# martinber/noaa-apt

Hardware: AMD Instinct MI355X
Metric: Msamples/sec WAV->APT-line decode (higher is better)
Workload: dtype f32; 1 GPU; synthetic 48000 Hz APT recording, 600 s (28800000 samples) per GPU, profile=standard: resample 13/50 (959 taps) -> AM envelope -> 37-tap low-pass -> sync correlation + peak picker -> 1198 rows x 2080 px; parallelism=1 GPU(s), 16 independent recordings per GPU and step, no collectives, recordings_per_call=16, mode=strict, rows=1198, n_sync=1199, input_resident_in_hbm=True, distinct_inputs_round_robin=16

## Files before the change

### noaa_apt_amd/csrc/apt_kernels_fused.hip

```cpp
#include "apt_kernels_fused_launch.hpp"

#include <hip/hip_runtime.h>

#include <cmath>
#include <cstdio>
#include <cstdlib>
#include <algorithm>
#include <cstring>
#include <type_traits>
#include <vector>

#pragma clang fp contract(off)

namespace apt::gpu {


bool fused_supported(uint32_t l, uint32_t m, uint32_t t1, uint32_t t2, uint32_t pw)
{
    if (l == 13 && m == 50 && t1 == 959 && t2 == 37 && pw == 3) return true;
    if (l == 13 && m == 100 && t1 == 1915 && t2 == 37 && pw == 3) return true;
    if (l == 13 && m == 30 && t1 == 2783 && t2 == 61 && pw == 5) return true;
    if (l == 13 && m == 60 && t1 == 5565 && t2 == 61 && pw == 5) return true;
    if (l == 13 && m == 75 && t1 == 639 && t2 == 43 && pw == 4) return true;
    return false;
}

uint32_t fused_group_size(uint32_t l) { return 4 * l; }

bool fused_takes_pcm16(uint32_t l, uint32_t m) { (void)l; return m % 2 == 0; }

uint32_t fused_tap_table_floats(uint32_t l, uint32_t m, uint32_t t1, int ch)
{
    (void)ch;
    const int li = static_cast<int>(l), mi = static_cast<int>(m), ti = static_cast<int>(t1);
    return static_cast<uint32_t>(fused_split_table_offset(li, mi, ti, 1) + (fused_split_nch(li, mi, ti, 1) + 1) * kSplitChunkDwords);
}

void fused_branch_taps(uint32_t l, uint32_t m, const float *coeff, uint32_t t1, int ch, float *hs, uint32_t t1_layout)
{
    (void)ch;
    if (t1_layout == 0) t1_layout = t1;
    const uint32_t tp = (t1_layout + l - 1) / l;
    const uint32_t clast = ((l - 1) * m + l - 1) / l;
    const uint32_t win = clast + tp;
    auto tap = [&](uint32_t b, int64_t q) -> float {
        const uint32_t cb = (b * m + l - 1) / l;
        const uint32_t pb = cb * l - b * m;
        if (q < static_cast<int64_t>(cb) || q >= static_cast<int64_t>(win)) return 0.f;
        const uint64_t j = pb + static_cast<uint64_t>(q - cb) * l;
        return j < t1 ? coeff[j] : 0.f;
    };
    const int li = static_cast<int>(l), mi = static_cast<int>(m), ti = static_cast<int>(t1_layout);
    for (int h = 0; h < 2; ++h) {
        const int b0 = fused_split_b0(li, h), nbr = fused_split_nbr(li, h), w0 = fused_split_w0(li, mi, h);
        const int nch_h = fused_split_nch(li, mi, ti, h);
        float *base = hs + fused_split_table_offset(li, mi, ti, h);
        for (int c = 0; c <= nch_h; ++c) {
            float *row = base + static_cast<size_t>(c) * kSplitChunkDwords;
            for (int i = 0; i < kSplitChunkDwords; ++i) row[i] = 0.f;
            if (c == nch_h) break;
            for (int e = 0; e < kSplitChunk; ++e) {
                const int64_t q = w0 + static_cast<int64_t>(kSplitChunk) * c + e;
                for (int k = 0; k < nbr / 2; ++k) {
                    row[6 * e + 2 * k] = tap(static_cast<uint32_t>(b0 + 2 * k), q);
                    row[6 * e + 2 * k + 1] = tap(static_cast<uint32_t>(b0 + 2 * k + 1), q);
                }
                if (nbr & 1) row[24 + e] = tap(static_cast<uint32_t>(b0 + nbr - 1), q);
            }
        }
    }
}

int fused_chunk_of(uint32_t m, bool fast)
{
    return fused_chunk(static_cast<int>(m), fast ? kModeFast : kModeStrict);
}

void fused_lowpass_pairs(const float *h2, uint32_t t2, float *h2p)
{
    for (uint32_t k = 0; k <= t2; ++k) {
        h2p[2 * k] = k >= 1 ? h2[k - 1] : 0.f;
        h2p[2 * k + 1] = k < t2 ? h2[k] : 0.f;
    }
}

uint32_t fused_f16_table_dwords(uint32_t l, uint32_t m, uint32_t t1)
{
    const uint32_t tp = (t1 + l - 1) / l;
    const uint32_t clast = ((l - 1) * m + l - 1) / l;
    return ((clast + tp + 1) / 2) * 16;
}

float fused_f16_branch_taps(uint32_t l, uint32_t m, const float *coeff, uint32_t t1, uint32_t *table)
{
    const uint32_t tp = (t1 + l - 1) / l;
    const uint32_t clast = ((l - 1) * m + l - 1) / l;
    const uint32_t win = clast + tp;
    auto tap = [&](uint32_t b, uint32_t q) -> float {
        const uint32_t cb = (b * m + l - 1) / l;
        const uint32_t pb = cb * l - b * m;
        if (q < cb || q >= win) return 0.f;
        const uint64_t j = pb + static_cast<uint64_t>(q - cb) * l;
        return j < t1 ? coeff[j] : 0.f;
    };
    float mx = 0.f;
    for (uint32_t j = 0; j < t1; ++j) mx = fmaxf(mx, fabsf(coeff[j]));
    int e = 0;
    if (mx > 0.f) (void)frexpf(mx, &e);
    const int sh = -e + 1;
    const float scale = ldexpf(1.f, sh);
    auto bits = [](float v) -> uint32_t {
        const _Float16 h = static_cast<_Float16>(v);
        uint16_t u;
        __builtin_memcpy(&u, &h, 2);
        return u;
    };
    const uint32_t nqp = (win + 1) / 2;
    for (uint32_t qp = 0; qp < nqp; ++qp)
        for (uint32_t b = 0; b < 16; ++b)
            table[qp * 16 + b] = b < l ? (bits(tap(b, 2 * qp) * scale) | (bits(tap(b, 2 * qp + 1) * scale) << 16)) : 0u;
    return ldexpf(1.f, -sh);
}

bool fused_f16_supported(uint32_t l, uint32_t m, uint32_t t1, uint32_t t2, uint32_t pw)
{
    return l == 13 && m == 50 && t1 == 959 && t2 == 37 && pw == 3;
}

float fused_gm_slack(uint32_t pw, float scale)
{
    return static_cast<float>(38u * pw - 1u + pw + 18u) * 1.03f * 0x1p-24f * 1.0001f * (scale >= 1.f ? scale : 1.f);
}

bool fused_fast_supported(uint32_t l, uint32_t m, uint32_t t1, uint32_t t2, uint32_t pw)
{
    if (l == 13 && m == 60 && t1 == 5565) return false;
    if (l == 13 && m == 75) return false;
    return fused_supported(l, m, t1, t2, pw);
}

uint32_t fused_pad_t2(uint32_t l, uint32_t m, uint32_t t2, uint32_t pw)
{
    if (l != 13 || pw != 3 || (m != 50 && m != 100)) return 0;
    if ((t2 & 1u) == 0 || t2 == 37 || t2 > static_cast<uint32_t>(kPadT2Max)) return 0;
    return static_cast<uint32_t>(kPadT2Max);
}
uint32_t fused_pad_t1(uint32_t l, uint32_t m, uint32_t t1, uint32_t t2, uint32_t pw)
{
    if (l != 13 || (t1 & 1u) == 0) return 0;
    uint32_t bound = 0;
    if ((t2 == 37 || fused_pad_t2(l, m, t2, pw) != 0) && pw == 3) bound = m == 50 ? kPadT1Max48k : m == 100 ? kPadT1Max96k : 0;
    else if (t2 == 61 && pw == 5) bound = m == 30 ? kPadT1Max48kSlow : m == 60 ? kPadT1Max96kSlow : 0;
    else if (t2 == 43 && pw == 4) bound = m == 75 ? kPadT1Max96kFastp : 0;
    return t1 <= bound ? bound : 0;
}

bool fused_mfma_supported(uint32_t l, uint32_t m, uint32_t t1, uint32_t t2, uint32_t pw)
{
    if (l != 13 || t2 != 37 || pw != 3 || (t1 & 1u) == 0) return false;
    if (m == 50) return t1 <= static_cast<uint32_t>(kMfmaT1Max48k);
    if (m == 100) return t1 <= static_cast<uint32_t>(kMfmaT1Max96k);
    return false;
}

namespace {
uint32_t mfma_kpad(uint32_t l, uint32_t m)
{
    const uint32_t t1max = m == 50 ? kMfmaT1Max48k : kMfmaT1Max96k;
    const uint32_t win = ((l - 1) * m + l - 1) / l + (t1max + l - 1) / l;
    return (win + 31u) / 32u * 32u;
}
template <typename At>
void mfma_fragments(At &&at, uint32_t nks, uint32_t *table)
{
    auto upper = [](float v) -> uint32_t {
        uint32_t u;
        __builtin_memcpy(&u, &v, 4);
        return u >> 16;
    };
    auto value = [](uint32_t h) -> float {
        const uint32_t u = h << 16;
        float v;
        __builtin_memcpy(&v, &u, 4);
        return v;
    };
    for (uint32_t s = 0; s < nks; ++s)
        for (uint32_t lane = 0; lane < 64; ++lane)
            for (uint32_t jp = 0; jp < 4; ++jp) {
                uint32_t w[3] = {0, 0, 0};
                for (uint32_t h = 0; h < 2; ++h) {
                    const float v = at(lane & 15u, 32u * s + 8u * (lane >> 4) + 2u * jp + h);
                    const uint32_t p0 = upper(v);
                    const float r1 = v - value(p0);
                    const uint32_t p1 = upper(r1);
                    const float r2 = r1 - value(p1);
                    const uint32_t p2 = upper(r2);
                    w[0] |= p0 << (16u * h);
                    w[1] |= p1 << (16u * h);
                    w[2] |= p2 << (16u * h);
                }
                for (uint32_t pc = 0; pc < 3; ++pc) table[((pc * nks + s) * 64u + lane) * 4u + jp] = w[pc];
            }
}
}

uint32_t fused_mfma_table_dwords(uint32_t l, uint32_t m) { return 3u * (mfma_kpad(l, m) / 32u) * 64u * 4u; }

void fused_mfma_table(uint32_t l, uint32_t m, const float *coeff, uint32_t t1, uint32_t *table)
{
    auto at = [&](uint32_t b, uint32_t q) -> float {
        if (b >= l) return 0.f;
        const uint32_t cb = (b * m + l - 1) / l, pb = cb * l - b * m;
        if (q < cb) return 0.f;
        const uint64_t j = pb + static_cast<uint64_t>(q - cb) * l;
        return j < t1 ? coeff[j] : 0.f;
    };
    mfma_fragments(at, mfma_kpad(l, m) / 32u, table);
}

bool fused_front_end(hipStream_t s, uint32_t l, uint32_t m, uint32_t t1, uint32_t t2, uint32_t pw, int mode,
                     bool pcm16, const CallArgs &call, const FusedParams *d_prm, uint64_t max_w, int lds_pad)
{
    if (call.count == 0 || call.count > static_cast<uint32_t>(kMaxCall)) return false;
// ... 479 lines not shown
```

### noaa_apt_amd/csrc/apt_kernels_fused_impl.hpp

```cpp
#pragma once

#include "apt_kernels_fused_launch.hpp"
#include "apt_envelope.hpp"
#include "apt_sync_corr.hpp"

#include <hip/hip_runtime.h>

#include <algorithm>
#include <atomic>
#include <cmath>
#include <cstdlib>
#include <type_traits>

#pragma clang fp contract(off)

#define APT_S1(n) "s" #n
#define APT_S8_(a, b, c, d, e, f, g, h) APT_S1(a), APT_S1(b), APT_S1(c), APT_S1(d), APT_S1(e), APT_S1(f), APT_S1(g), APT_S1(h)
#define APT_S8(n) APT_S8_X(n)
#define APT_S16(n) APT_S16_X(n)
#define APT_S8_X(n) APT_S8_##n
#define APT_S16_X(n) APT_S16_##n
#define APT_S8_52 APT_S8_(52, 53, 54, 55, 56, 57, 58, 59)
#define APT_S16_36 APT_S8_(36, 37, 38, 39, 40, 41, 42, 43), APT_S8_(44, 45, 46, 47, 48, 49, 50, 51)
#define APT_S16_64 APT_S8_(64, 65, 66, 67, 68, 69, 70, 71), APT_S8_(72, 73, 74, 75, 76, 77, 78, 79)
// ... 787 lines not shown
        for (int b = 0; b < L; ++b) r[b] = (kq + b < k_lo || kq + b >= k_hi) ? 0.f : acc[b] * f16_unscale;
    } else if constexpr (MFMA) {
        static_assert(Gm::SPLIT && L <= 16 && M % 2 == 0 && Gm::XSHIFT % 2 == 0, "windows start on sample pairs");
        constexpr int NS = Gm::NS, NKS = Gm::KPAD / 32, PLANE = Gm::XT_PAD / 2;
        constexpr int NGW = NS / 16 / (NTHR / 64);
        static_assert(NGW * 16 * (NTHR / 64) == NS, "whole groups per wave");
        uint32_t *l32 = reinterpret_cast<uint32_t *>(lds);
        uint32_t *nf_flag = l32 + 2 * PLANE;
        const int lane = tid & 63, wave = tid >> 6;
        typedef uint32_t u4m __attribute__((ext_vector_type(4)));
        typedef __bf16 b8m __attribute__((ext_vector_type(8)));
        auto as_b8 = [](u4m v) -> b8m { return __builtin_bit_cast(b8m, v); };
        typedef const u4m __attribute__((address_space(1))) *gu4_ptr;
        const gu4_ptr atab = (gu4_ptr)(prm->hs) + lane;
        if (tid == 0) *nf_flag = 0u;
        auto planes_to_lds = [&](const XReg (&xv)[NXR]) {
#pragma unroll
            for (int e = 0; e < NXR; ++e) {
                const int q = (tid + e * kFusedThreads) * 4;
                if (q < Gm::XT_PAD) {
                    float v[4];
                    if constexpr (sizeof(XT) == 4) {
                        v[0] = xv[e].x, v[1] = xv[e].y, v[2] = xv[e].z, v[3] = xv[e].w;
                    } else {
                        v[0] = static_cast<float>(static_cast<int16_t>(xv[e].x & 0xFFFFu)), v[1] = static_cast<float>(static_cast<int32_t>(xv[e].x) >> 16);
                        v[2] = static_cast<float>(static_cast<int16_t>(xv[e].y & 0xFFFFu)), v[3] = static_cast<float>(static_cast<int32_t>(xv[e].y) >> 16);
                    }
                    float r[4];
#pragma unroll
                    for (int i = 0; i < 4; ++i) r[i] = v[i] - __uint_as_float(__float_as_uint(v[i]) & 0xFFFF0000u);
                    const u2 w0 = (u2){__builtin_amdgcn_perm(__float_as_uint(v[1]), __float_as_uint(v[0]), 0x07060302u),
                                       __builtin_amdgcn_perm(__float_as_uint(v[3]), __float_as_uint(v[2]), 0x07060302u)};
                    const u2 w1 = (u2){__builtin_amdgcn_perm(__float_as_uint(r[1]), __float_as_uint(r[0]), 0x07060302u),
                                       __builtin_amdgcn_perm(__float_as_uint(r[3]), __float_as_uint(r[2]), 0x07060302u)};
                    *reinterpret_cast<u2 *>(l32 + q / 2) = w0;
                    *reinterpret_cast<u2 *>(l32 + PLANE + q / 2) = w1;
                }
            }
        };
        f4 racc[2][NGW];
        auto mfma_sub = [&](auto subc) {
            constexpr int SUB = decltype(subc)::value;
            int base[NGW];
#pragma unroll
            for (int g = 0; g < NGW; ++g) {
                racc[SUB][g] = (f4){0.f, 0.f, 0.f, 0.f};
                const int wl = (wave * NGW + g) * 16 + (lane & 15);
                base[g] = wl * (M / 2) + Gm::XSHIFT / 2 + 4 * (lane >> 4);
            }
            u4m an0 = atab[0], an1 = atab[NKS * 64], an2 = atab[2 * NKS * 64];
#pragma unroll
            for (int s_ = 0; s_ < NKS; ++s_) {
                const u4m a0 = an0, a1 = an1, a2 = an2;
                if (s_ + 1 < NKS) {
                    an0 = atab[(s_ + 1) * 64];
                    an1 = atab[(NKS + s_ + 1) * 64];
                    an2 = atab[(2 * NKS + s_ + 1) * 64];
                }
                u4m b0[NGW], b1[NGW];
#pragma unroll
                for (int g = 0; g < NGW; ++g) {
                    const uint32_t *bp = l32 + base[g] + 16 * s_;
                    b0[g] = (u4m){bp[0], bp[1], bp[2], bp[3]};
                    b1[g] = (u4m){bp[PLANE], bp[PLANE + 1], bp[PLANE + 2], bp[PLANE + 3]};
                }
#pragma unroll
                for (int g = 0; g < NGW; ++g) racc[SUB][g] = __builtin_amdgcn_mfma_f32_16x16x32_bf16(as_b8(a2), as_b8(b0[g]), racc[SUB][g], 0, 0, 0);
#pragma unroll
                for (int g = 0; g < NGW; ++g) racc[SUB][g] = __builtin_amdgcn_mfma_f32_16x16x32_bf16(as_b8(a1), as_b8(b1[g]), racc[SUB][g], 0, 0, 0);
#pragma unroll
                for (int g = 0; g < NGW; ++g) racc[SUB][g] = __builtin_amdgcn_mfma_f32_16x16x32_bf16(as_b8(a1), as_b8(b0[g]), racc[SUB][g], 0, 0, 0);
#pragma unroll
                for (int g = 0; g < NGW; ++g) racc[SUB][g] = __builtin_amdgcn_mfma_f32_16x16x32_bf16(as_b8(a0), as_b8(b1[g]), racc[SUB][g], 0, 0, 0);
#pragma unroll
                for (int g = 0; g < NGW; ++g) racc[SUB][g] = __builtin_amdgcn_mfma_f32_16x16x32_bf16(as_b8(a0), as_b8(b0[g]), racc[SUB][g], 0, 0, 0);
                __builtin_amdgcn_sched_barrier(0);
            }
        };
        XReg xr1[NXR];
        planes_to_lds(xr);
        __builtin_amdgcn_sched_barrier(0);
        load_tile(ri, tile, 1, xr1);
        __syncthreads();
        mfma_sub(std::integral_constant<int, 0>{});
        __syncthreads();
        planes_to_lds(xr1);
        __syncthreads();
        mfma_sub(std::integral_constant<int, 1>{});
        APT_MARK("END stage1");
        {
            float sum = 0.f;
#pragma unroll
            for (int sub = 0; sub < 2; ++sub)
#pragma unroll
                for (int g = 0; g < NGW; ++g) sum += (racc[sub][g].x + racc[sub][g].y) + (racc[sub][g].z + racc[sub][g].w);
            if ((__float_as_uint(sum) & 0x7F800000u) == 0x7F800000u) *nf_flag = 1u;
        }
        __syncthreads();
        const bool tile_nf = *nf_flag != 0u;
        {
#pragma unroll
            for (int sub = 0; sub < 2; ++sub)
#pragma unroll
                for (int g = 0; g < NGW; ++g) {
                    const int wdw = sub * NS + (wave * NGW + g) * 16 + (lane & 15);
#pragma unroll
                    for (int rr_ = 0; rr_ < 4; ++rr_) {
                        const int b = 4 * (lane >> 4) + rr_;
                        if (b < L) P[wdw * L + b] = racc[sub][g][rr_];
                    }
                }
        }
        if (tile_nf) {
            __syncthreads();
            const XT *__restrict__ xg = static_cast<const XT *>(call.rec[ri].x);
            const uint64_t n_in = call.rec[ri].n;
            const float *__restrict__ cf = prm->coeff;
            const uint32_t t1r = prm->t1;
            for (int b = 0; b < L; ++b) {
                const int64_t k = (tile * Gm::OWN_K - Gm::PRE_K) + kq + b;
                float sum = 0.f;
                if (k >= 0) {
                    const uint64_t v = static_cast<uint64_t>(k) * static_cast<uint64_t>(M);
                    uint64_t x0 = (v + L - 1) / L;
                    for (uint64_t j = x0 * L - v; j < t1r; j += L, ++x0)
                        if (x0 < n_in) sum = __builtin_fmaf(cf[j], static_cast<float>(xg[x0]), sum);
                }
                P[tid * L + b] = sum;
            }
        }
        __syncthreads();
#pragma unroll
        for (int b = 0; b < L; ++b) r[b] = P[tid * L + b];
        if (!interior) {
            bool any = false;
#pragma unroll
            for (int b = 0; b < L; ++b)
                if (kq + b < k_lo || kq + b >= k_hi) {
                    r[b] = 0.f;
                    any = true;
                }
            if (any) {
#pragma unroll
                for (int b = 0; b < L; ++b) P[tid * L + b] = r[b];
            }
            __syncthreads();
        }
    } else if constexpr (Gm::SPLIT) {
        static_assert(L == 13 && Gm::XSHIFT % 2 == 0 && (M % 2 == 0 || sizeof(XT) == 4),
                      "SPLIT: halves of 7 and 6 branches (three pairs each); window reads of aligned sample pairs, or — odd M, f32 input only — of single samples");
        constexpr bool WIDE = M % 4 == 0 && Gm::XSHIFT % 4 == 0;
        constexpr int NS = Gm::NS;
        const int wl = tid & (NS - 1);
        constexpr int NH0 = fused_split_nbr(L, 0);
        float rh[2][NH0];
        if constexpr (PAD) {
#pragma unroll
            for (int j = 0; j < NH0; ++j) rh[0][j] = rh[1][j] = 0.f;
        }
        auto half = [&](auto hc, auto subc) {
            constexpr int H = decltype(hc)::value, SUB = decltype(subc)::value;
            constexpr int B0 = fused_split_b0(L, H), NBR = fused_split_nbr(L, H);
            constexpr int NPH = NBR / 2;
            constexpr bool ODDH = (NBR & 1) != 0;
            static_assert(NPH == 3, "three branch pairs per half");
            constexpr int W0 = fused_split_w0(L, M, H), NCH = fused_split_nch(L, M, T1, H);
            constexpr int CHW = kSplitChunkDwords;
            const cf2_ptr hsp = hs + fused_split_table_offset(L, M, T1, H) / 2;
            typedef uint32_t u16s __attribute__((ext_vector_type(16)));
            typedef uint32_t u8s __attribute__((ext_vector_type(8)));
            typedef uint32_t u4s __attribute__((ext_vector_type(4)));
            u16s ta[2];
            u8s tb[2];
            u4s tc[2];
            typedef float f4w __attribute__((ext_vector_type(4)));
            using XRaw = std::conditional_t<sizeof(XT) == 4, f4w, u2>;
            XRaw xraw[2];
            f2 acc[NPH];
            float accl = 0.f;
#pragma unroll
            for (int k = 0; k < NPH; ++k) acc[k] = (f2){0.f, 0.f};
            auto issue = [&](auto cc) {
                constexpr int c = decltype(cc)::value;
                if constexpr ((c & 1) == 0)
                    asm volatile("s_load_dwordx16 s[36:51], %0, %1\n\ts_load_dwordx8 s[52:59], %0, %2\n\ts_load_dwordx4 s[60:63], %0, %3"
                                 :: "s"(hsp), "n"(c * CHW * 4), "n"(c * CHW * 4 + 64), "n"(c * CHW * 4 + 96)
                                 : APT_S16(36), APT_S8(52), APT_S4_60);
                else
                    asm volatile("s_load_dwordx16 s[64:79], %0, %1\n\ts_load_dwordx8 s[80:87], %0, %2\n\ts_load_dwordx4 s[88:91], %0, %3"
                                 :: "s"(hsp), "n"(c * CHW * 4), "n"(c * CHW * 4 + 64), "n"(c * CHW * 4 + 96)
                                 : APT_S16(64), APT_S8(80), APT_S4_88);
                constexpr int q0 = Gm::XSHIFT + W0 + kSplitChunk * c;
                if constexpr (sizeof(XT) == 4) {
                    if constexpr (WIDE) {
                        xraw[c & 1] = *reinterpret_cast<const f4w *>(P + wl * M + q0);
                    } else if constexpr (M % 2 != 0) {
                        const float *wp = P + wl * M + q0;
                        xraw[c & 1] = (f4w){wp[0], wp[1], wp[2], wp[3]};
                    } else {
                        const f2 lo = *reinterpret_cast<const f2 *>(P + wl * M + q0), hi = *reinterpret_cast<const f2 *>(P + wl * M + q0 + 2);
                        xraw[c & 1] = (f4w){lo.x, lo.y, hi.x, hi.y};
                    }
                } else if constexpr (WIDE) {
                    xraw[c & 1] = *reinterpret_cast<const u2 *>(reinterpret_cast<const int16_t *>(lds) + wl * M + q0);
                } else {
                    const uint32_t *w32 = reinterpret_cast<const uint32_t *>(lds) + (wl * M + q0) / 2;
                    xraw[c & 1] = (u2){w32[0], w32[1]};
                }
            };
            auto wait_taps = [&](auto cc) {
                constexpr int c = decltype(cc)::value;
                u16s &ra = ta[c & 1];
                u8s &rb = tb[c & 1];
                u4s &rc = tc[c & 1];
                XRaw &xr_ = xraw[c & 1];
                if constexpr ((c & 1) == 0)
                    asm volatile("s_waitcnt lgkmcnt(0)" : "={s[36:51]}"(ra), "={s[52:59]}"(rb), "={s[60:63]}"(rc), "+v"(xr_));
                else
                    asm volatile("s_waitcnt lgkmcnt(0)" : "={s[64:79]}"(ra), "={s[80:87]}"(rb), "={s[88:91]}"(rc), "+v"(xr_));
            };
            auto tapd = [&](auto cc, auto ii) -> float {
                constexpr int buf = decltype(cc)::value & 1, i = decltype(ii)::value;
                if constexpr (i < 16) return __uint_as_float(ta[buf][i]);
                else if constexpr (i < 24) return __uint_as_float(tb[buf][i - 16]);
                else return __uint_as_float(tc[buf][i - 24]);
            };
            issue(std::integral_constant<int, 0>{});
            static_for<0, NCH>([&](auto cc) {
                constexpr int c = decltype(cc)::value;
                wait_taps(cc);
                __builtin_amdgcn_sched_barrier(0);
                if constexpr (c + 1 < NCH) issue(std::integral_constant<int, c + 1>{});
                __builtin_amdgcn_sched_barrier(0);
                f4w xv;
                if constexpr (sizeof(XT) == 4) {
                    xv = xraw[c & 1];
                } else {
                    const u2 u = xraw[c & 1];
                    xv = (f4w){static_cast<float>(static_cast<int16_t>(u.x & 0xFFFFu)), static_cast<float>(static_cast<int32_t>(u.x) >> 16),
                               static_cast<float>(static_cast<int16_t>(u.y & 0xFFFFu)), static_cast<float>(static_cast<int32_t>(u.y) >> 16)};
                }
                static_for<0, kSplitChunk>([&](auto ee) {
                    constexpr int e = decltype(ee)::value;
                    constexpr int q = W0 + kSplitChunk * c + e;
                    const float xq = xv[e];
                    const f2 xpair_e = (e < 2) ? __builtin_shufflevector(xv, xv, 0, 1) : __builtin_shufflevector(xv, xv, 2, 3);
                    auto mul_bcast = [&](f2 t) -> f2 {
                        f2 p;
                        if constexpr ((e & 1) == 0) asm("v_pk_mul_f32 %0, %1, %2 op_sel_hi:[0,1]" : "=v"(p) : "v"(xpair_e), "s"(t));
                        else asm("v_pk_mul_f32 %0, %1, %2 op_sel:[1,0]" : "=v"(p) : "v"(xpair_e), "s"(t));
                        return p;
                    };
                    auto fma_bcast = [&](f2 t, f2 a) -> f2 {
                        if constexpr ((e & 1) == 0) asm("v_pk_fma_f32 %0, %1, %2, %0 op_sel_hi:[0,1,1]" : "+v"(a) : "v"(xpair_e), "s"(t));
                        else asm("v_pk_fma_f32 %0, %1, %2, %0 op_sel:[1,0,0]" : "+v"(a) : "v"(xpair_e), "s"(t));
                        return a;
                    };
                    f2 pr[NPH];
                    static_for<0, NPH>([&](auto kk) {
                        constexpr int k = decltype(kk)::value;
                        constexpr bool va = branch_uses<L, M, T1>(B0 + 2 * k, q), vb = branch_uses<L, M, T1>(B0 + 2 * k + 1, q);
                        const f2 t = (f2){tapd(cc, std::integral_constant<int, 6 * e + 2 * k>{}), tapd(cc, std::integral_constant<int, 6 * e + 2 * k + 1>{})};
                        pr[k] = (f2){0.f, 0.f};
                        if constexpr (FAST) {
                            if constexpr (va && vb) acc[k] = fma_bcast(t, acc[k]);
                            else if constexpr (va) acc[k].x = __builtin_fmaf(t.x, xq, acc[k].x);
                            else if constexpr (vb) acc[k].y = __builtin_fmaf(t.y, xq, acc[k].y);
                        } else {
                            if constexpr (va && vb) pr[k] = mul_bcast(t);
                            else if constexpr (va) pr[k].x = t.x * xq;
                            else if constexpr (vb) pr[k].y = t.y * xq;
                        }
                    });
                    if constexpr (!FAST) {
                        static_for<0, NPH>([&](auto kk) {
                            constexpr int k = decltype(kk)::value;
                            constexpr bool va = branch_uses<L, M, T1>(B0 + 2 * k, q), vb = branch_uses<L, M, T1>(B0 + 2 * k + 1, q);
                            if constexpr (va && vb) acc[k] = acc[k] + pr[k];
                            else if constexpr (va) acc[k].x = acc[k].x + pr[k].x;
                            else if constexpr (vb) acc[k].y = acc[k].y + pr[k].y;
                        });
                    }
                });
                if constexpr (ODDH) {
                    static_for<0, kSplitChunk / 2>([&](auto pp) {
                        constexpr int e = 2 * decltype(pp)::value;
                        constexpr int q = W0 + kSplitChunk * c + e;
                        constexpr bool u0 = branch_uses<L, M, T1>(B0 + NBR - 1, q), u1 = branch_uses<L, M, T1>(B0 + NBR - 1, q + 1);
                        const f2 t = (f2){tapd(cc, std::integral_constant<int, 24 + e>{}), tapd(cc, std::integral_constant<int, 25 + e>{})};
                        const f2 xp = (f2){xv[e], xv[e + 1]};
                        if constexpr (FAST) {
                            if constexpr (u0) accl = __builtin_fmaf(t.x, xp.x, accl);
                            if constexpr (u1) accl = __builtin_fmaf(t.y, xp.y, accl);
                        } else if constexpr (u0 && u1) {
                            const f2 po = t * xp;
                            accl = accl + po.x;
                            accl = accl + po.y;
                        } else if constexpr (u0) {
                            accl = accl + t.x * xp.x;
                        } else if constexpr (u1) {
                            accl = accl + t.y * xp.y;
                        }
                    });
                }
                static_for<0, NPH>([&](auto kk) {
                    f2 &a = acc[decltype(kk)::value];
                    asm volatile("" : "+v"(a));
                });
                asm volatile("" : "+v"(accl));
                __builtin_amdgcn_sched_barrier(0);
            });
#pragma unroll
            for (int k = 0; k < NPH; ++k) {
                rh[SUB][2 * k] = acc[k].x;
                rh[SUB][2 * k + 1] = acc[k].y;
            }
            if constexpr (ODDH) rh[SUB][NBR - 1] = accl;
        };
        const bool first_half = (tid < NS) != ((tile & 1) != 0);
        [[maybe_unused]] uint32_t *pad_flag = reinterpret_cast<uint32_t *>(lds) + (Gm::XT_LDS - 4);
        if constexpr (PAD && sizeof(XT) == 4) {
            if (tid == 0) *pad_flag = 0u;
        }
        if constexpr (PADLP && sizeof(XT) == 4) {
            if (tid == 0) reinterpret_cast<uint32_t *>(lds)[Gm::LP_FLAG_OFF] = 0u;
        }
        XReg xr1[NXR];
        load_tile(ri, tile, 1, xr1);
        if (first_half) half(std::integral_constant<int, 0>{}, std::integral_constant<int, 0>{});
        else half(std::integral_constant<int, 1>{}, std::integral_constant<int, 0>{});
        __syncthreads();
        tile_to_lds(xr1);
        __syncthreads();
        if (first_half) half(std::integral_constant<int, 0>{}, std::integral_constant<int, 1>{});
        else half(std::integral_constant<int, 1>{}, std::integral_constant<int, 1>{});
        APT_MARK("END stage1");
        if constexpr (PAD && sizeof(XT) == 4) {
            float chk = 0.f;
#pragma unroll
            for (int j = 0; j < fused_split_nbr(L, 0); ++j) chk = chk + (rh[0][j] + rh[1][j]);
            if ((__float_as_uint(chk) & 0x7F800000u) == 0x7F800000u) *pad_flag = 1u;
        }
        __syncthreads();
        if (first_half) {
#pragma unroll
            for (int j = 0; j < fused_split_nbr(L, 0); ++j) {
                P[wl * L + j] = rh[0][j];
                P[(NS + wl) * L + j] = rh[1][j];
            }
        } else {
#pragma unroll
            for (int j = 0; j < fused_split_nbr(L, 1); ++j) {
                P[wl * L + fused_split_b0(L, 1) + j] = rh[0][j];
                P[(NS + wl) * L + fused_split_b0(L, 1) + j] = rh[1][j];
            }
        }
        if constexpr (PAD && sizeof(XT) == 4) {
            static_assert(Gm::XT_LDS - 4 >= Gm::TILE_K, "the flag lies behind R");
            if (*pad_flag != 0u) {
                __syncthreads();
                const XT *__restrict__ xg = static_cast<const XT *>(call.rec[ri].x);
                const uint64_t n_in = call.rec[ri].n;
                const float *__restrict__ cf = prm->coeff;
                const uint32_t t1r = prm->t1;
                for (int b = 0; b < L; ++b) {
                    const int64_t k = (tile * Gm::OWN_K - Gm::PRE_K) + kq + b;
                    float sum = 0.f;
                    if (k >= 0) {
                        const uint64_t v = static_cast<uint64_t>(k) * static_cast<uint64_t>(M);
                        uint64_t x0 = (v + L - 1) / L;
                        for (uint64_t j = x0 * L - v; j < t1r; j += L, ++x0)
                            if (x0 < n_in) sum = sum + cf[j] * static_cast<float>(xg[x0]);
                    }
                    P[tid * L + b] = sum;
                }
            }
        }
        __syncthreads();
#pragma unroll
        for (int b = 0; b < L; ++b) r[b] = P[tid * L + b];
        if (!interior) {
            bool any = false;
#pragma unroll
            for (int b = 0; b < L; ++b)
                if (kq + b < k_lo || kq + b >= k_hi) {
                    r[b] = 0.f;
                    any = true;
                }
            if (any) {
#pragma unroll
                for (int b = 0; b < L; ++b) P[tid * L + b] = r[b];
            }
            __syncthreads();
        }
    } else {
        static_assert(Gm::SPLIT || F16, "the specialised kernels are 256-thread workgroups");
    }
    APT_MARK("BEGIN r_store");
    if constexpr (!Gm::SPLIT) {
    __syncthreads();
#pragma unroll
    for (int b = 0; b < L; ++b) P[tid * L + b] = r[b];
    __syncthreads();
    }
    after_tile_in_lds();
    }

    if constexpr (APT_FUSED_STOP == 2) return;
    typedef const FusedParams APT_CONST_AS *cprm_ptr;
    cprm_ptr late = (cprm_ptr)(prm);
    asm volatile("" : "+s"(late));
    const float cosphi2 = late->cosphi2, sinphi = late->sinphi;
    const float inv_sinphi = late->inv_sinphi;
    const cfloat_ptr h2 = (cfloat_ptr)(late->h2);
    const cf2_ptr h2p = (cf2_ptr)(late->h2p);
    typedef const SlotPtrs APT_CONST_AS *cslot_ptr;
    const cslot_ptr slots = (cslot_ptr)(late->slots);
    const int want_gm = late->want_gm;
    const float gm_slack = late->gm_slack;
    APT_MARK("END r_store");

    auto envelope = [&](auto interior_tag) {
    constexpr bool INT = decltype(interior_tag)::value;
    if constexpr (FAST) {
        float prev = (tid > 0) ? P[tid * L - 1] : 0.f;
        if constexpr (INT) {
            const f2 cos2 = (f2){cosphi2, cosphi2}, inv2 = (f2){inv_sinphi, inv_sinphi};
#pragma unroll
            for (int p2 = 0; p2 < (L + 1) / 2; ++p2) {
                const f2 A = (f2){r[2 * p2], (2 * p2 + 1 < L) ? r[2 * p2 + 1] : r[2 * p2]};
                const f2 S = p2 == 0 ? (f2){prev, r[0]} : (f2){P[tid * L + 2 * p2 - 1], P[tid * L + 2 * p2]};
                const f2 rad = __builtin_elementwise_fma(-(S * A), cos2, (S * S) + (A * A));
                const f2 q = (f2){__builtin_amdgcn_sqrtf(rad.x), __builtin_amdgcn_sqrtf(rad.y)} * inv2;
                Q[tid * L + 2 * p2] = q.x;
                if (2 * p2 + 1 < L) Q[tid * L + 2 * p2 + 1] = q.y;
            }
        } else {
        float prev_sq = prev * prev;
#pragma unroll
        for (int b = 0; b < L; ++b) {
            const float curr = r[b];
            const float curr_sq = curr * curr;
            const float rad = __builtin_fmaf(-(prev * curr), cosphi2, prev_sq + curr_sq);
            Q[tid * L + b] = (kq + b > k_lo) ? __builtin_amdgcn_sqrtf(rad) * inv_sinphi : 0.f;
            prev = curr;
            prev_sq = curr_sq;
        }
        }
    } else {
        float cosv = cosphi2, sinv = sinphi, invv = inv_sinphi;
        asm volatile("" : "+v"(cosv), "+v"(sinv), "+v"(invv));
        float prev = (tid > 0) ? P[tid * L - 1] : 0.f;
        float xr[L];
        bool in_range = inv_sinphi != 0.f;
        if constexpr (INT) {
            APT_MARK("BEGIN envelope_radicands");
            constexpr int NPE = (L + 1) / 2;
            f2 rad[NPE];
            uint32_t umin = 0xFFFFFFFFu, umax = 0u;
            const f2 cos2 = (f2){cosv, cosv};
#pragma unroll
            for (int p2 = 0; p2 < NPE; ++p2) {
                const f2 A = (f2){r[2 * p2], (2 * p2 + 1 < L) ? r[2 * p2 + 1] : r[2 * p2]};
                const f2 S = p2 == 0 ? (f2){prev, r[0]} : (f2){P[tid * L + 2 * p2 - 1], P[tid * L + 2 * p2]};
                const f2 ss = (S * S) + (A * A);
                const f2 cc = (S * A) * cos2;
                rad[p2] = ss - cc;
                const uint32_t u0 = __float_as_uint(rad[p2].x), u1 = __float_as_uint(rad[p2].y);
                umin = u0 < umin ? u0 : umin;
                umin = u1 < umin ? u1 : umin;
                umax = u0 > umax ? u0 : umax;
                umax = u1 > umax ? u1 : umax;
            }
            in_range = in_range && umin >= 0x0F800000u && umax <= 0x71800000u;
            APT_MARK("END envelope_radicands");
            if (__all(in_range)) {
                APT_MARK("BEGIN envelope_roots");
                const f2 sin2 = (f2){sinv, sinv}, inv2 = (f2){invv, invv}, half2 = (f2){0.5f, 0.5f};
#pragma unroll
                for (int p2 = 0; p2 < NPE; ++p2) {
                    const f2 x = rad[p2];
                    const f2 y = (f2){__builtin_amdgcn_rsqf(x.x), __builtin_amdgcn_rsqf(x.y)};
                    const f2 g = x * y;
                    const f2 h = half2 * y;
                    const f2 d = __builtin_elementwise_fma(-g, g, x);
                    const f2 root = __builtin_elementwise_fma(d, h, g);
                    const f2 q0 = root * inv2;
                    const f2 rem = __builtin_elementwise_fma(-sin2, q0, root);
                    const f2 q = __builtin_elementwise_fma(rem, inv2, q0);
                    Q[tid * L + 2 * p2] = q.x;
                    if (2 * p2 + 1 < L) Q[tid * L + 2 * p2 + 1] = q.y;
                }
                APT_MARK("END envelope_roots");
            } else {
#pragma unroll
                for (int b = 0; b < L; ++b) {
                    const float x = (b & 1) ? rad[b / 2].y : rad[b / 2].x;
// ... 496 lines not shown
```

### noaa_apt_amd/csrc/apt_kernels_fused_launch.hpp

```cpp
#pragma once

#include "apt_kernels.hpp"

namespace apt::gpu {

constexpr int kModeStrict = 0;
constexpr int kModeF16Taps = 1;
constexpr int kModeFast = 2;
constexpr int kModeMfma = 3;
constexpr int kModeStrictPad = 4;
#ifndef APT_PHASE_HALVES
#define APT_PHASE_HALVES 1
#endif
constexpr bool phase_halves(int nq, bool stream, int nthr, int t2, bool fast)
{
    return APT_PHASE_HALVES != 0 && nq == 1 && !stream && nthr == 256 && !(fast && t2 == 37);
}
constexpr int kModeStrictPad2 = 5;
constexpr int kPadT2Max = 45;
constexpr int fused_geom_var(int mode)
{
    return mode == kModeF16Taps ? 1 : mode == kModeMfma ? 2 : (mode == kModeStrictPad || mode == kModeStrictPad2) ? 3 : 0;
}
constexpr int kPadT1Max48k = 1079, kPadT1Max96k = 2145;
constexpr int kPadT1Max48kSlow = 3133, kPadT1Max96kSlow = 6253, kPadT1Max96kFastp = 727;
constexpr int kMfmaT1Max48k = 1053, kMfmaT1Max96k = 2119;

constexpr int fused_chunk(int m, int mode)
{
    return 4;
}

constexpr int kSplitChunk = 4, kSplitChunkDwords = 28;
constexpr int fused_branch_first(int l, int m, int b) { return (b * m + l - 1) / l; }
constexpr int fused_branch_end(int l, int m, int t1, int b)
{
    const int cb = fused_branch_first(l, m, b), pb = cb * l - b * m;
    return cb + (t1 - pb + l - 1) / l;
}
constexpr int fused_split_b0(int l, int h) { return h == 0 ? 0 : (l + 1) / 2; }
constexpr int fused_split_nbr(int l, int h) { return h == 0 ? (l + 1) / 2 : l / 2; }
constexpr int fused_split_w0(int l, int m, int h) { return fused_branch_first(l, m, fused_split_b0(l, h)) / 4 * 4; }
constexpr int fused_split_nch(int l, int m, int t1, int h)
{
    int end = 0;
    for (int b = fused_split_b0(l, h); b < fused_split_b0(l, h) + fused_split_nbr(l, h); ++b)
        end = fused_branch_end(l, m, t1, b) > end ? fused_branch_end(l, m, t1, b) : end;
    return (end - fused_split_w0(l, m, h) + kSplitChunk - 1) / kSplitChunk;
}
constexpr int fused_split_table_offset(int l, int m, int t1, int h)
{
    return h == 0 ? 0 : (fused_split_nch(l, m, t1, 0) + 1) * kSplitChunkDwords;
}

struct FusedLaunch {
    hipStream_t s;
    const CallArgs *call;
    const FusedParams *prm;
    uint64_t max_w;
    size_t table_lds_floats;
    int lds_pad = 0;
};

void fused_launch_48k_f32(const FusedLaunch &a);
void fused_launch_48k_i16(const FusedLaunch &a);
void fused_launch_96k_f32(const FusedLaunch &a);
void fused_launch_96k_i16(const FusedLaunch &a);
void fused_launch_48k_f16taps_f32(const FusedLaunch &a);
void fused_launch_48k_f16taps_i16(const FusedLaunch &a);
void fused_launch_48k_fast_f32(const FusedLaunch &a);
void fused_launch_48k_fast_i16(const FusedLaunch &a);
void fused_launch_96k_fast_f32(const FusedLaunch &a);
void fused_launch_96k_fast_i16(const FusedLaunch &a);
void fused_launch_48k_mfma_f32(const FusedLaunch &a);
void fused_launch_48k_mfma_i16(const FusedLaunch &a);
void fused_launch_96k_mfma_f32(const FusedLaunch &a);
void fused_launch_96k_mfma_i16(const FusedLaunch &a);
void fused_launch_48k_pad_f32(const FusedLaunch &a);
void fused_launch_48k_pad_i16(const FusedLaunch &a);
void fused_launch_96k_pad_f32(const FusedLaunch &a);
void fused_launch_96k_pad_i16(const FusedLaunch &a);
void fused_launch_48k_slow_pad_f32(const FusedLaunch &a);
void fused_launch_48k_slow_pad_i16(const FusedLaunch &a);
void fused_launch_96k_slow_pad_f32(const FusedLaunch &a);
void fused_launch_96k_slow_pad_i16(const FusedLaunch &a);
void fused_launch_96k_fastp_pad_f32(const FusedLaunch &a);
void fused_launch_48k_pad2_f32(const FusedLaunch &a);
void fused_launch_48k_pad2_i16(const FusedLaunch &a);
void fused_launch_96k_pad2_f32(const FusedLaunch &a);
void fused_launch_96k_pad2_i16(const FusedLaunch &a);
void fused_launch_phase_std_pad2_f32(const FusedLaunch &a);
void fused_launch_phase_std_pad2_i16(const FusedLaunch &a);
void fused_launch_phase2_std_pad2_f32(const FusedLaunch &a);
void fused_launch_phase2_std_pad2_i16(const FusedLaunch &a);
void fused_launch_phase4_std_pad2_f32(const FusedLaunch &a);
void fused_launch_phase4_std_pad2_i16(const FusedLaunch &a);
void fused_launch_48k_slow_f32(const FusedLaunch &a);
void fused_launch_48k_slow_i16(const FusedLaunch &a);
void fused_launch_48k_slow_fast_f32(const FusedLaunch &a);
void fused_launch_48k_slow_fast_i16(const FusedLaunch &a);
void fused_launch_96k_slow_f32(const FusedLaunch &a);
void fused_launch_96k_slow_i16(const FusedLaunch &a);
void fused_launch_96k_fastp_f32(const FusedLaunch &a);
void fused_launch_phase_fastp_f32(const FusedLaunch &a);
void fused_launch_phase_fastp_i16(const FusedLaunch &a);
void fused_launch_phase_fastp_fast_f32(const FusedLaunch &a);
void fused_launch_phase_fastp_fast_i16(const FusedLaunch &a);
void fused_launch_tab_std_f32(const FusedLaunch &a);
void fused_launch_tab_std_i16(const FusedLaunch &a);
void fused_launch_tab_std_fast_f32(const FusedLaunch &a);
void fused_launch_tab_std_fast_i16(const FusedLaunch &a);
void fused_launch_phase_std_f32(const FusedLaunch &a);
void fused_launch_phase_std_i16(const FusedLaunch &a);
void fused_launch_phase_std_fast_f32(const FusedLaunch &a);
void fused_launch_phase_std_fast_i16(const FusedLaunch &a);
void fused_launch_phase512_std_f32(const FusedLaunch &a);
void fused_launch_phase512_std_i16(const FusedLaunch &a);
void fused_launch_phase512_std_fast_f32(const FusedLaunch &a);
void fused_launch_phase512_std_fast_i16(const FusedLaunch &a);
void fused_launch_phase2_std_f32(const FusedLaunch &a);
void fused_launch_phase2_std_i16(const FusedLaunch &a);
void fused_launch_phase2_std_fast_f32(const FusedLaunch &a);
void fused_launch_phase2_std_fast_i16(const FusedLaunch &a);
void fused_launch_phase4_std_f32(const FusedLaunch &a);
void fused_launch_phase4_std_i16(const FusedLaunch &a);
void fused_launch_phase4_std_fast_f32(const FusedLaunch &a);
void fused_launch_phase4_std_fast_i16(const FusedLaunch &a);
void fused_launch_phase4_fastp_f32(const FusedLaunch &a);
void fused_launch_phase4_fastp_i16(const FusedLaunch &a);
void fused_launch_phase8_fastp_f32(const FusedLaunch &a);
void fused_launch_phase8_fastp_i16(const FusedLaunch &a);
void fused_launch_phase16_fastp_f32(const FusedLaunch &a);
void fused_launch_phase16_fastp_i16(const FusedLaunch &a);
void fused_launch_phase_slowp_f32(const FusedLaunch &a);
void fused_launch_phase_slowp_i16(const FusedLaunch &a);
void fused_launch_phase2_slowp_f32(const FusedLaunch &a);
void fused_launch_phase2_slowp_i16(const FusedLaunch &a);
void fused_launch_phase4_slowp_f32(const FusedLaunch &a);
void fused_launch_phase4_slowp_i16(const FusedLaunch &a);
void fused_launch_phase1024_std_f32(const FusedLaunch &a);
void fused_launch_phase1024_std_i16(const FusedLaunch &a);
void fused_launch_phase1024_std_fast_f32(const FusedLaunch &a);
void fused_launch_phase1024_std_fast_i16(const FusedLaunch &a);
#ifdef APT_WITH_PROBES
void fused_launch_probe1(const FusedLaunch &a);
void fused_launch_probe2(const FusedLaunch &a);
void fused_launch_probe3(const FusedLaunch &a);
void fused_launch_probe4(const FusedLaunch &a);
void fused_launch_probe5(const FusedLaunch &a);
void fused_launch_probe11(const FusedLaunch &a);
void fused_launch_probe12(const FusedLaunch &a);
void fused_launch_probe13(const FusedLaunch &a);
void fused_launch_probe14(const FusedLaunch &a);
void fused_launch_probe15(const FusedLaunch &a);
void fused_launch_probe16(const FusedLaunch &a);
void fused_launch_probe8(const FusedLaunch &a);
void fused_launch_probe9(const FusedLaunch &a);
void fused_launch_probe17(const FusedLaunch &a);
#endif

}
```

Before: 543,800 Msamples/s.

## Split 13 polyphase branches into two 6-branch halves plus a separate odd-branch wave

For the 48 kHz strict f32 profile, the split polyphase resampler now gives each half of the block exactly six branches (three packed pairs). The thirteenth branch goes to one rotating wave, which computes it with packed multiplies over paired LDS reads. This removes the unpaired scalar branch from one half and the extra tap-table loads, which should balance the two halves. The cost is a third table region and a host layout that is more complex, plus extra work on one wave per tile that may add imbalance.

Result: slower. 524,500 Msamples/s (-3.5%).

```diff
diff --git a/noaa_apt_amd/csrc/apt_kernels_fused.hip b/noaa_apt_amd/csrc/apt_kernels_fused.hip
--- a/noaa_apt_amd/csrc/apt_kernels_fused.hip
+++ b/noaa_apt_amd/csrc/apt_kernels_fused.hip
@@ -33,7 +33,8 @@
 {
     (void)ch;
     const int li = static_cast<int>(l), mi = static_cast<int>(m), ti = static_cast<int>(t1);
-    return static_cast<uint32_t>(fused_split_table_offset(li, mi, ti, 1) + (fused_split_nch(li, mi, ti, 1) + 1) * kSplitChunkDwords);
+    if (fused_split_oddpair(li, mi, ti, kModeStrict, 4)) return static_cast<uint32_t>(fused_oddpair_table_floats(li, mi, ti));
+    return static_cast<uint32_t>(fused_split_table_floats(li, mi, ti));
 }
 
 void fused_branch_taps(uint32_t l, uint32_t m, const float *coeff, uint32_t t1, int ch, float *hs, uint32_t t1_layout)
@@ -69,6 +70,24 @@
             }
         }
     }
+    if (!fused_split_oddpair(li, mi, ti, kModeStrict, 4)) return;
+    for (int h = 0; h < 2; ++h) {
+        const int b0 = fused_oddpair_b0(li, h), w0 = fused_oddpair_w0(li, mi, h);
+        const int nch_h = fused_oddpair_nch(li, mi, ti, h);
+        float *base = hs + fused_oddpair_table_offset(li, mi, ti, h);
+        for (int c = 0; c <= nch_h; ++c) {
+            float *row = base + static_cast<size_t>(c) * kOddPairChunkDwords;
+            for (int i = 0; i < kOddPairChunkDwords; ++i) row[i] = 0.f;
+            if (c == nch_h) break;
+            for (int e = 0; e < kSplitChunk; ++e)
+                for (int k = 0; k < li / 2; ++k)
+                    row[6 * e + k] = tap(static_cast<uint32_t>(b0 + k), w0 + static_cast<int64_t>(kSplitChunk) * c + e);
+        }
+    }
+    float *run = hs + fused_oddpair_table_offset(li, mi, ti, 2);
+    const int c_last = fused_branch_first(li, mi, li - 1), n_last = fused_oddpair_ntaps(li, mi, ti);
+    for (int i = 0; i < fused_oddpair_table_floats(li, mi, ti) - fused_oddpair_table_offset(li, mi, ti, 2); ++i)
+        run[i] = i < n_last ? tap(l - 1, c_last + i) : 0.f;
 }
 
 int fused_chunk_of(uint32_t m, bool fast)
diff --git a/noaa_apt_amd/csrc/apt_kernels_fused_impl.hpp b/noaa_apt_amd/csrc/apt_kernels_fused_impl.hpp
--- a/noaa_apt_amd/csrc/apt_kernels_fused_impl.hpp
+++ b/noaa_apt_amd/csrc/apt_kernels_fused_impl.hpp
@@ -963,7 +963,9 @@
         constexpr bool WIDE = M % 4 == 0 && Gm::XSHIFT % 4 == 0;
         constexpr int NS = Gm::NS;
         const int wl = tid & (NS - 1);
-        constexpr int NH0 = fused_split_nbr(L, 0);
+        constexpr bool OP = fused_split_oddpair(L, M, T1, MODE, static_cast<int>(sizeof(XT)));
+        static_assert(!OP || (!PAD && !FAST && NS == 128 && M % 2 == 0), "odd-pair form: strict, exact tap count, two waves of windows");
+        constexpr int NH0 = OP ? L / 2 : fused_split_nbr(L, 0);
         float rh[2][NH0];
         if constexpr (PAD) {
 #pragma unroll
@@ -971,13 +973,14 @@
         }
         auto half = [&](auto hc, auto subc) {
             constexpr int H = decltype(hc)::value, SUB = decltype(subc)::value;
-            constexpr int B0 = fused_split_b0(L, H), NBR = fused_split_nbr(L, H);
+            constexpr int B0 = OP ? fused_oddpair_b0(L, H) : fused_split_b0(L, H), NBR = OP ? L / 2 : fused_split_nbr(L, H);
             constexpr int NPH = NBR / 2;
             constexpr bool ODDH = (NBR & 1) != 0;
             static_assert(NPH == 3, "three branch pairs per half");
-            constexpr int W0 = fused_split_w0(L, M, H), NCH = fused_split_nch(L, M, T1, H);
-            constexpr int CHW = kSplitChunkDwords;
-            const cf2_ptr hsp = hs + fused_split_table_offset(L, M, T1, H) / 2;
+            constexpr int W0 = OP ? fused_oddpair_w0(L, M, H) : fused_split_w0(L, M, H);
+            constexpr int NCH = OP ? fused_oddpair_nch(L, M, T1, H) : fused_split_nch(L, M, T1, H);
+            constexpr int CHW = OP ? kOddPairChunkDwords : kSplitChunkDwords;
+            const cf2_ptr hsp = hs + (OP ? fused_oddpair_table_offset(L, M, T1, H) : fused_split_table_offset(L, M, T1, H)) / 2;
             typedef uint32_t u16s __attribute__((ext_vector_type(16)));
             typedef uint32_t u8s __attribute__((ext_vector_type(8)));
             typedef uint32_t u4s __attribute__((ext_vector_type(4)));
@@ -993,7 +996,15 @@
             for (int k = 0; k < NPH; ++k) acc[k] = (f2){0.f, 0.f};
             auto issue = [&](auto cc) {
                 constexpr int c = decltype(cc)::value;
-                if constexpr ((c & 1) == 0)
+                if constexpr (OP && (c & 1) == 0)
+                    asm volatile("s_load_dwordx16 s[36:51], %0, %1\n\ts_load_dwordx8 s[52:59], %0, %2"
+                                 :: "s"(hsp), "n"(c * CHW * 4), "n"(c * CHW * 4 + 64)
+                                 : APT_S16(36), APT_S8(52));
+                else if constexpr (OP)
+                    asm volatile("s_load_dwordx16 s[64:79], %0, %1\n\ts_load_dwordx8 s[80:87], %0, %2"
+                                 :: "s"(hsp), "n"(c * CHW * 4), "n"(c * CHW * 4 + 64)
+                                 : APT_S16(64), APT_S8(80));
+                else if constexpr ((c & 1) == 0)
                     asm volatile("s_load_dwordx16 s[36:51], %0, %1\n\ts_load_dwordx8 s[52:59], %0, %2\n\ts_load_dwordx4 s[60:63], %0, %3"
                                  :: "s"(hsp), "n"(c * CHW * 4), "n"(c * CHW * 4 + 64), "n"(c * CHW * 4 + 96)
                                  : APT_S16(36), APT_S8(52), APT_S4_60);
@@ -1023,9 +1034,13 @@
                 constexpr int c = decltype(cc)::value;
                 u16s &ra = ta[c & 1];
                 u8s &rb = tb[c & 1];
-                u4s &rc = tc[c & 1];
+                [[maybe_unused]] u4s &rc = tc[c & 1];
                 XRaw &xr_ = xraw[c & 1];
-                if constexpr ((c & 1) == 0)
+                if constexpr (OP && (c & 1) == 0)
+                    asm volatile("s_waitcnt lgkmcnt(0)" : "={s[36:51]}"(ra), "={s[52:59]}"(rb), "+v"(xr_));
+                else if constexpr (OP)
+                    asm volatile("s_waitcnt lgkmcnt(0)" : "={s[64:79]}"(ra), "={s[80:87]}"(rb), "+v"(xr_));
+                else if constexpr ((c & 1) == 0)
                     asm volatile("s_waitcnt lgkmcnt(0)" : "={s[36:51]}"(ra), "={s[52:59]}"(rb), "={s[60:63]}"(rc), "+v"(xr_));
                 else
                     asm volatile("s_waitcnt lgkmcnt(0)" : "={s[64:79]}"(ra), "={s[80:87]}"(rb), "={s[88:91]}"(rc), "+v"(xr_));
@@ -1128,6 +1143,68 @@
             }
             if constexpr (ODDH) rh[SUB][NBR - 1] = accl;
         };
+        [[maybe_unused]] f2 ro[2];
+        [[maybe_unused]] auto odd = [&](auto subc) {
+            constexpr int SUB = decltype(subc)::value;
+            constexpr int C0 = branch_first<L, M>(L - 1), NT = fused_oddpair_ntaps(L, M, T1);
+            constexpr int OC = kOddChunk, NOC = (NT + OC - 1) / OC;
+            static_assert(OC == 4 && C0 + NT <= Gm::WIN, "one s_load_dwordx4 per chunk; the run ends inside the window");
+            static_assert(NT - 1 + M <= 255 && NS == 128, "both windows' samples within one two-address read's offsets; 64 window pairs");
+            const cf2_ptr hop = hs + fused_oddpair_table_offset(L, M, T1, 2) / 2;
+            const uint32_t xa = static_cast<uint32_t>(reinterpret_cast<uintptr_t>((__attribute__((address_space(3))) float *)(P))) +
+                                static_cast<uint32_t>(((tid & 63) * 2 * M + (Gm::XSHIFT + C0)) * 4);
+            typedef uint32_t u4s __attribute__((ext_vector_type(4)));
+            u4s to[2];
+            f2 xp[2][OC];
+            f2 acc = (f2){0.f, 0.f};
+            auto issue = [&](auto cc) {
+                constexpr int c = decltype(cc)::value;
+                if constexpr ((c & 1) == 0)
+                    asm volatile("s_load_dwordx4 s[60:63], %0, %1" :: "s"(hop), "n"(c * OC * 4) : APT_S4_60);
+                else
+                    asm volatile("s_load_dwordx4 s[88:91], %0, %1" :: "s"(hop), "n"(c * OC * 4) : APT_S4_88);
+                static_for<0, OC>([&](auto ee) {
+                    constexpr int i = c * OC + decltype(ee)::value;
+                    f2 &dst = xp[c & 1][decltype(ee)::value];
+                    const uint32_t adr = xa;
+                    if constexpr (i < NT) asm volatile("ds_read2_b32 %0, %1 offset0:%2 offset1:%3" : "=v"(dst) : "v"(adr), "n"(i), "n"(i + M));
+                    else asm volatile("" : "=v"(dst));
+                });
+            };
+            auto wait_taps = [&](auto cc) {
+                constexpr int c = decltype(cc)::value;
+                u4s &r = to[c & 1];
+                f2(&x)[OC] = xp[c & 1];
+                if constexpr ((c & 1) == 0)
+                    asm volatile("s_waitcnt lgkmcnt(0)" : "={s[60:63]}"(r), "+v"(x[0]), "+v"(x[1]), "+v"(x[2]), "+v"(x[3]));
+                else
+                    asm volatile("s_waitcnt lgkmcnt(0)" : "={s[88:91]}"(r), "+v"(x[0]), "+v"(x[1]), "+v"(x[2]), "+v"(x[3]));
+            };
+            issue(std::integral_constant<int, 0>{});
+            static_for<0, NOC>([&](auto cc) {
+                constexpr int c = decltype(cc)::value;
+                wait_taps(cc);
+                __builtin_amdgcn_sched_barrier(0);
+                if constexpr (c + 1 < NOC) issue(std::integral_constant<int, c + 1>{});
+                __builtin_amdgcn_sched_barrier(0);
+                f2 pr[OC];
+                static_for<0, OC / 2>([&](auto pp) {
+                    constexpr int e = 2 * decltype(pp)::value, i = c * OC + e;
+                    const f2 t = (f2){__uint_as_float(to[c & 1][e]), __uint_as_float(to[c & 1][e + 1])};
+                    f2 &p0 = pr[e], &p1 = pr[e + 1];
+                    const f2 x0 = xp[c & 1][e], x1 = xp[c & 1][e + 1];
+                    if constexpr (i < NT) asm("v_pk_mul_f32 %0, %1, %2 op_sel_hi:[1,0]" : "=v"(p0) : "v"(x0), "s"(t));
+                    if constexpr (i + 1 < NT) asm("v_pk_mul_f32 %0, %1, %2 op_sel:[0,1]" : "=v"(p1) : "v"(x1), "s"(t));
+                });
+                static_for<0, OC>([&](auto ee) {
+                    if constexpr (c * OC + decltype(ee)::value < NT) acc = acc + pr[decltype(ee)::value];
+                });
+                asm volatile("" : "+v"(acc));
+                __builtin_amdgcn_sched_barrier(0);
+            });
+            ro[SUB] = acc;
+        };
+        [[maybe_unused]] const bool odd_wave = __builtin_amdgcn_readfirstlane(tid >> 6) == static_cast<int>(tile & 3);
         const bool first_half = (tid < NS) != ((tile & 1) != 0);
         [[maybe_unused]] uint32_t *pad_flag = reinterpret_cast<uint32_t *>(lds) + (Gm::XT_LDS - 4);
         if constexpr (PAD && sizeof(XT) == 4) {
@@ -1140,11 +1217,17 @@
         load_tile(ri, tile, 1, xr1);
         if (first_half) half(std::integral_constant<int, 0>{}, std::integral_constant<int, 0>{});
         else half(std::integral_constant<int, 1>{}, std::integral_constant<int, 0>{});
+        if constexpr (OP) {
+            if (odd_wave) odd(std::integral_constant<int, 0>{});
+        }
         __syncthreads();
         tile_to_lds(xr1);
         __syncthreads();
         if (first_half) half(std::integral_constant<int, 0>{}, std::integral_constant<int, 1>{});
         else half(std::integral_constant<int, 1>{}, std::integral_constant<int, 1>{});
+        if constexpr (OP) {
+            if (odd_wave) odd(std::integral_constant<int, 1>{});
+        }
         APT_MARK("END stage1");
         if constexpr (PAD && sizeof(XT) == 4) {
             float chk = 0.f;
@@ -1153,7 +1236,21 @@
             if ((__float_as_uint(chk) & 0x7F800000u) == 0x7F800000u) *pad_flag = 1u;
         }
         __syncthreads();
-        if (first_half) {
+        if constexpr (OP) {
+            const int b0 = first_half ? 0 : fused_oddpair_b0(L, 1);
+#pragma unroll
+            for (int j = 0; j < L / 2; ++j) {
+                P[wl * L + b0 + j] = rh[0][j];
+                P[(NS + wl) * L + b0 + j] = rh[1][j];
+            }
+            if (odd_wave) {
+                const int wa = 2 * (tid & 63);
+                P[wa * L + (L - 1)] = ro[0].x;
+                P[(wa + 1) * L + (L - 1)] = ro[0].y;
+                P[(NS + wa) * L + (L - 1)] = ro[1].x;
+                P[(NS + wa + 1) * L + (L - 1)] = ro[1].y;
+            }
+        } else if (first_half) {
 #pragma unroll
             for (int j = 0; j < fused_split_nbr(L, 0); ++j) {
                 P[wl * L + j] = rh[0][j];
diff --git a/noaa_apt_amd/csrc/apt_kernels_fused_launch.hpp b/noaa_apt_amd/csrc/apt_kernels_fused_launch.hpp
--- a/noaa_apt_amd/csrc/apt_kernels_fused_launch.hpp
+++ b/noaa_apt_amd/csrc/apt_kernels_fused_launch.hpp
@@ -51,6 +51,36 @@
 constexpr int fused_split_table_offset(int l, int m, int t1, int h)
 {
     return h == 0 ? 0 : (fused_split_nch(l, m, t1, 0) + 1) * kSplitChunkDwords;
+}
+constexpr int fused_split_table_floats(int l, int m, int t1)
+{
+    return fused_split_table_offset(l, m, t1, 1) + (fused_split_nch(l, m, t1, 1) + 1) * kSplitChunkDwords;
+}
+
+constexpr int kOddPairChunkDwords = 24, kOddChunk = 4;
+constexpr bool fused_split_oddpair(int l, int m, int t1, int mode, int xbytes)
+{
+    return l == 13 && m == 50 && t1 == 959 && mode == kModeStrict && xbytes == 4;
+}
+constexpr int fused_oddpair_b0(int l, int h) { return h * (l / 2); }
+constexpr int fused_oddpair_w0(int l, int m, int h) { return fused_branch_first(l, m, fused_oddpair_b0(l, h)) / 4 * 4; }
+constexpr int fused_oddpair_nch(int l, int m, int t1, int h)
+{
+    int end = 0;
+    for (int b = fused_oddpair_b0(l, h); b < fused_oddpair_b0(l, h) + l / 2; ++b)
+        end = fused_branch_end(l, m, t1, b) > end ? fused_branch_end(l, m, t1, b) : end;
+    return (end - fused_oddpair_w0(l, m, h) + kSplitChunk - 1) / kSplitChunk;
+}
+constexpr int fused_oddpair_ntaps(int l, int m, int t1) { return fused_branch_end(l, m, t1, l - 1) - fused_branch_first(l, m, l - 1); }
+constexpr int fused_oddpair_table_offset(int l, int m, int t1, int h)
+{
+    int off = fused_split_table_floats(l, m, t1);
+    for (int i = 0; i < h; ++i) off += (fused_oddpair_nch(l, m, t1, i) + 1) * kOddPairChunkDwords;
+    return off;
+}
+constexpr int fused_oddpair_table_floats(int l, int m, int t1)
+{
+    return fused_oddpair_table_offset(l, m, t1, 2) + ((fused_oddpair_ntaps(l, m, t1) + kOddChunk - 1) / kOddChunk + 1) * kOddChunk;
 }
 
 struct FusedLaunch {
```
